# stjude-rust-labs/ngs

Measured on AMD Instinct MI355X. Metric: BAM records/sec (whole node), all qc facets, 150 bp reads, higher is better.
Workload: dtype u8/u32 integer (u64 accumulators)

## Files before the change

ngs_amd/csrc/cov_stream.hip:

```cpp
#include <hip/hip_runtime.h>

#include <type_traits>

#include "kernels.h"

namespace ngsq {

typedef unsigned long long u64;

constexpr uint32_t ST_THREADS = 256;
constexpr uint32_t ST_WAVES = ST_THREADS / 64;
constexpr uint32_t ST_W = 1024;
constexpr uint32_t ST_LIST = 232;
constexpr uint32_t ST_HOT_BINS = 64, ST_HOT_REP = 4, ST_HOT = ST_HOT_BINS * ST_HOT_REP;

__device__ __forceinline__ u64 st_key(int32_t rf, int32_t ps) {
    return rf < 0 ? 0xFFFFFFFF00000000ull : ((u64)(uint32_t)rf << 32) | (uint32_t)(ps + 1);
}
__device__ __forceinline__ bool st_valid(const DeviceState &st, int32_t rf, int32_t ps) {
    return rf >= 0 && (uint32_t)rf < st.n_refs && ps >= 0 && st.ref_depth_off[rf] != NO_DEPTH;
}

__global__ __launch_bounds__(256) void k_cov_plan_tiles(DeviceState st, DeviceBatch b, CovStreamArgs a) {
    NGSQ_FOREGROUND_WAVE();
    const uint64_t n_wt = (b.n + CS_TILE - 1) / CS_TILE;
    const uint64_t t = (uint64_t)blockIdx.x * blockDim.x + threadIdx.x;
    if (t == 0) {
        const u64 k0 = st_key(b.ref_id[0], b.pos[0]);
        if (k0 < *a.last_key) atomicAdd(&st.counters[C_COV_UNSORTED], 1ull);
        *a.last_key = st_key(b.ref_id[b.n - 1], b.pos[b.n - 1]);
    }
    const uint32_t lane = threadIdx.x & 63u;
    auto first_of = [&](int64_t u, int32_t &r, int32_t &p) {
        const bool ok = u >= 0 && (uint64_t)u < n_wt;
        r = ok ? b.ref_id[(uint64_t)u * CS_TILE] : -1;
        p = ok ? b.pos[(uint64_t)u * CS_TILE] : -1;
    };
    int32_t rf[4], ps[4];
    first_of((int64_t)t, rf[1], ps[1]);
    rf[0] = __shfl_up(rf[1], 1, 64), ps[0] = __shfl_up(ps[1], 1, 64);
    rf[2] = __shfl_down(rf[1], 1, 64), ps[2] = __shfl_down(ps[1], 1, 64);
    rf[3] = __shfl_down(rf[1], 2, 64), ps[3] = __shfl_down(ps[1], 2, 64);
    if (lane == 0) first_of((int64_t)t - 1, rf[0], ps[0]);
    if (lane == 63) first_of((int64_t)t + 1, rf[2], ps[2]);
    if (lane >= 62) first_of((int64_t)t + 2, rf[3], ps[3]);
    if (t >= n_wt) return;
    auto streamable = [&](int k) {
        return st_valid(st, rf[k], ps[k]) && rf[k + 1] == rf[k] && ps[k + 1] >= 0;
    };
    if (!streamable(1)) return;
    const bool prev_same = streamable(0) && rf[0] == rf[1];
    const bool next_same = streamable(2) && rf[2] == rf[1];
    if (!prev_same) atomicMin(&a.plan_a[rf[1]], (uint32_t)ps[1] + 1);
    if (!next_same) atomicMax(&a.plan_z[rf[1]], (uint32_t)ps[2] + 1);
}

__global__ __launch_bounds__(256) void k_cov_plan_refs(DeviceState st, CovStreamArgs a) {
    NGSQ_FOREGROUND_WAVE();
    const uint32_t r = blockIdx.x * blockDim.x + threadIdx.x;
    if (r == 0 && a.span_next) *a.span_next = 0;
    if (r >= st.n_refs) return;
    const uint32_t pa = a.plan_a[r], pz = a.plan_z[r], prev = a.prev_end[r];
    const uint32_t acc = st.end_acc[r];
    uint32_t guard = a.guard_until[r];
    if (a.head_guard && guard == 0 && (pa != CS_NONE || acc != 0)) {
        const uint64_t g = (uint64_t)(pa != CS_NONE ? pa : acc) + a.head_guard;
        guard = g > 0xFFFFFFFEull ? 0xFFFFFFFEu : (uint32_t)g;
        a.guard_until[r] = guard;
    }
    uint32_t H = CS_NONE, T = CS_NONE;
    if (pa != CS_NONE && pz > pa) {
        uint64_t base = pa > prev + 1 ? pa : (uint64_t)prev + 1;
        if (guard > base) base = guard;
        const uint64_t h = (base + COV_CHUNK - 1) / COV_CHUNK * COV_CHUNK;
        const uint64_t lim = pz < (uint64_t)st.ref_len[r] + 1 ? pz : (uint64_t)st.ref_len[r] + 1;
        const uint64_t tt = lim / COV_CHUNK * COV_CHUNK;
        if (h < tt) {
            H = (uint32_t)h;
            T = (uint32_t)tt;
        }
    }
    a.plan_h[r] = H;
    a.plan_t[r] = T;
    a.prev_end[r] = acc > prev ? acc : prev;
    a.plan_a[r] = CS_NONE;
    a.plan_z[r] = 0;
}

__device__ __forceinline__ uint32_t st_wave_scan(uint32_t v) {
    v += (uint32_t)__builtin_amdgcn_update_dpp(0, (int)v, 0x111, 0xF, 0xF, false);
    v += (uint32_t)__builtin_amdgcn_update_dpp(0, (int)v, 0x112, 0xF, 0xF, false);
    v += (uint32_t)__builtin_amdgcn_update_dpp(0, (int)v, 0x114, 0xF, 0xF, false);
    v += (uint32_t)__builtin_amdgcn_update_dpp(0, (int)v, 0x118, 0xF, 0xF, false);
    v += (uint32_t)__builtin_amdgcn_update_dpp(0, (int)v, 0x142, 0xA, 0xF, false);
    v += (uint32_t)__builtin_amdgcn_update_dpp(0, (int)v, 0x143, 0xC, 0xF, false);
    return v;
}
__device__ __forceinline__ uint32_t st_wave_max(uint32_t v) {
#pragma unroll
    for (int o = 32; o > 0; o >>= 1) v = max(v, (uint32_t)__shfl_xor(v, o, 64));
    return v;
}

__host__ __device__ inline uint32_t st_hist_words(uint32_t cov_cap) { return ((cov_cap + 2 + 1) / 2 + 3) & ~3u; }

constexpr uint32_t ST_PER_LANE = 8;
constexpr uint32_t ST_PASS = 64 * ST_PER_LANE;
static_assert(ST_W % ST_PASS == 0, "whole passes");

struct StTileIn {
    int4 p;
    uint4 c;
    int32_t rf_t, ps_t, rf_n, ps_n;
};

constexpr uint32_t ST_MIN_BLOCKS = 4;
__global__ __launch_bounds__(ST_THREADS, ST_MIN_BLOCKS) void k_cov_stream(DeviceState st, DeviceBatch b, CovStreamArgs a) {
    NGSQ_FOREGROUND_WAVE();
    extern __shared__ __attribute__((aligned(16))) uint32_t s_dyn[];
    const uint32_t nb = a.cov_cap + 2;
    const uint32_t tid = threadIdx.x, lane = tid & 63;
    const uint32_t wave = (uint32_t)__builtin_amdgcn_readfirstlane((int)(tid >> 6));
    const uint32_t hw = st_hist_words(a.cov_cap);
    uint32_t *const win = s_dyn + wave * (ST_W + hw + ST_HOT + ST_LIST);
    uint32_t *const hist = win + ST_W;
    uint32_t *const hot = hist + hw;
    uint32_t *const lst = hot + ST_HOT;
    for (uint32_t i = lane; i < ST_W + hw + ST_HOT + ST_LIST; i += 64) win[i] = 0;
    __builtin_amdgcn_fence(__ATOMIC_ACQ_REL, "wavefront");
    __builtin_amdgcn_wave_barrier();

    const uint64_t n_wt = (b.n + CS_TILE - 1) / CS_TILE;
    const uint64_t n_full = b.n / CS_TILE;
    const uint64_t n_units = (uint64_t)gridDim.x * ST_WAVES, unit = (uint64_t)blockIdx.x * ST_WAVES + wave;
    const uint64_t per = (n_wt + n_units - 1) / n_units;
    const uint64_t t_begin = per * unit < n_wt ? per * unit : n_wt;
    const uint64_t t_end = t_begin + per < n_wt ? t_begin + per : n_wt;
    const uint32_t maxspan = *st.batch_span;

    uint32_t hot_base = 0;
    int32_t hist_ref = -1;
    uint32_t since_flush = 0;
    u64 zero_run = 0;
    uint32_t lane_zero = 0;
    u64 *bins = a.bin_totals;
    u64 lane_bin = 0;
    uint32_t bin_q = 0, bin_p0 = 1, bin_p1 = 0;
    u64 t_lo = ~0ull, t_hi = 0;
    bool lst_valid = false;
    uint64_t lst_tile = 0;
    int32_t lst_ref = -1;
    uint32_t lst_lo = 0, lst_n = 0;
    int32_t plan_ref = -1;
    uint32_t pH = CS_NONE, pT = CS_NONE, pL = 0;
    uint64_t pOff = 0;

    auto flush_bin = [&]() {
        u64 v = lane_bin;
#pragma unroll
        for (int o = 32; o > 0; o >>= 1) v += __shfl_xor(v, o, 64);
        if (lane == 0 && v) atomicAdd(&bins[bin_q], v);
        lane_bin = 0;
    };
    auto flush_hot = [&]() {
        static_assert((ST_HOT_REP == 4 || ST_HOT_REP == 8) && ST_HOT_BINS <= 64, "one or two uint4 per lane");
        uint4 *const cell = reinterpret_cast<uint4 *>(hot) + (lane < ST_HOT_BINS ? lane : 0u) * (ST_HOT_REP / 4);
        uint32_t t = 0;
        if (lane < ST_HOT_BINS) {
#pragma unroll
            for (uint32_t q = 0; q < ST_HOT_REP / 4; q++) {
                const uint4 v = cell[q];
                cell[q] = make_uint4(0, 0, 0, 0);
                t += v.x + v.y + v.z + v.w;
            }
        }
        const uint32_t depth = hot_base + lane;
        const uint32_t bin = depth <= a.cov_cap ? depth : a.cov_cap + 1;
        if (t) atomicAdd(&hist[bin < hw ? bin : bin - hw], bin < hw ? t : t << 16);
        __builtin_amdgcn_fence(__ATOMIC_ACQ_REL, "wavefront");
        __builtin_amdgcn_wave_barrier();
    };
    auto flush_hist = [&]() {
        if (hist_ref < 0) return;
        flush_hot();
        u64 *dst = a.hist + (u64)hist_ref * nb;
        for (uint32_t i = lane; i < hw; i += 64) {
            const uint32_t v = hist[i];
            if (v) {
                if ((v & 0xFFFFu) && i < nb) atomicAdd(&dst[i], (u64)(v & 0xFFFFu));
                if ((v >> 16) && i + hw < nb) atomicAdd(&dst[i + hw], (u64)(v >> 16));
                hist[i] = 0;
            }
        }
        {
            u64 z = lane_zero;
#pragma unroll
            for (int o = 32; o > 0; o >>= 1) z += __shfl_xor(z, o, 64);
            if (lane == 0 && zero_run + z) atomicAdd(&dst[0], zero_run + z);
        }
        zero_run = 0;
        lane_zero = 0;
        since_flush = 0;
        __builtin_amdgcn_fence(__ATOMIC_ACQ_REL, "wavefront");
        __builtin_amdgcn_wave_barrier();
    };
    auto chunk_add = [&](bool active, uint64_t chunk, uint32_t val) {
        const u64 m = __ballot(active);
        if (!m) return;
        const uint32_t c0 = __shfl((uint32_t)chunk, __ffsll((long long)m) - 1, 64);
        const bool same = active && (uint32_t)chunk == c0;
        uint32_t sum = same ? val : 0u;
#pragma unroll
        for (int o = 32; o > 0; o >>= 1) sum += __shfl_xor(sum, o, 64);
        if (lane == 0 && sum) atomicAdd(&st.chunk_sums[c0], sum);
        if (active && !same) atomicAdd(&st.chunk_sums[chunk], val);
    };
    auto classic = [&](bool on, uint64_t off, uint32_t q0, uint32_t q1, bool minus_in_sum_only) {
        const uint64_t g0 = off + q0, g1 = off + q1;
        if (on) {
            atomicAdd(&st.depth[g0], 1u);
            if (!minus_in_sum_only) atomicAdd(&st.depth[g1], 0xFFFFFFFFu);
            t_lo = g0 < t_lo ? g0 : t_lo;
            t_hi = g1 + 1 > t_hi ? g1 + 1 : t_hi;
        }
        chunk_add(on, g0 / COV_CHUNK, 1u);
        chunk_add(on, g1 / COV_CHUNK, 0xFFFFFFFFu);
    };
    auto outside = [&](bool on, uint64_t off, uint32_t sj, uint32_t ej, uint32_t H, uint32_t T) {
        const bool head = on && sj < H;
        const uint32_t m = ej < H ? ej : H;
        if (__ballot(head)) classic(head, off, sj, m, m == H);
        const bool tl = on && T != CS_NONE && ej > T;
        if (__ballot(tl)) classic(tl, off, sj > T ? sj : T, ej, false);
    };

    auto load_full = [&](uint64_t t) -> StTileIn {
        const uint64_t base = t * CS_TILE, r0 = base + (uint64_t)lane * 4;
        StTileIn in;
        in.p = *reinterpret_cast<const int4 *>(b.pos + r0);
        in.c = *reinterpret_cast<const uint4 *>(st.cov_end + r0);
        const uint64_t nx = base + CS_TILE < b.n ? base + CS_TILE : base;
        in.rf_t = b.ref_id[base];
        in.ps_t = b.pos[base];
        in.rf_n = b.ref_id[nx];
        in.ps_n = b.pos[nx];
        return in;
    };

    auto process = [&](const StTileIn &in, uint64_t t) {
        const uint64_t base = t * CS_TILE;
        const uint64_t r0 = base + (uint64_t)lane * 4;
        const uint32_t s[4] = {(uint32_t)in.p.x + 1, (uint32_t)in.p.y + 1, (uint32_t)in.p.z + 1, (uint32_t)in.p.w + 1};
        const uint32_t e[4] = {in.c.x, in.c.y, in.c.z, in.c.w};
        const int32_t rf_t = __builtin_amdgcn_readfirstlane(in.rf_t), ps_t = __builtin_amdgcn_readfirstlane(in.ps_t);
        const int32_t rf_n = __builtin_amdgcn_readfirstlane(in.rf_n), ps_n = __builtin_amdgcn_readfirstlane(in.ps_n);
        const bool cand = base + CS_TILE < b.n && rf_t >= 0 && (uint32_t)rf_t < st.n_refs && ps_t >= 0 && rf_n == rf_t && ps_n >= 0;
        if (cand && rf_t != plan_ref) {
            plan_ref = rf_t;
            pH = (uint32_t)__builtin_amdgcn_readfirstlane((int)a.plan_h[rf_t]);
            pT = (uint32_t)__builtin_amdgcn_readfirstlane((int)a.plan_t[rf_t]);
            pL = (uint32_t)__builtin_amdgcn_readfirstlane((int)st.ref_len[rf_t]);
            const uint64_t o = st.ref_depth_off[rf_t];
            pOff = ((uint64_t)(uint32_t)__builtin_amdgcn_readfirstlane((int)(o >> 32)) << 32) |
                   (uint32_t)__builtin_amdgcn_readfirstlane((int)(uint32_t)o);
        }
        const bool streamable = cand && pOff != NO_DEPTH;
        const uint32_t H = streamable ? pH : CS_NONE, T = streamable ? pT : CS_NONE, Lr = pL;
        const uint64_t off = pOff;

        if (streamable) {
#pragma unroll
            for (uint32_t j = 0; j < 4; j++) {
                const uint32_t ej = e[j] < Lr + 1 ? e[j] : Lr + 1;
                const bool on = e[j] != 0 && s[j] < ej && (s[j] < H || ej > T);
                if (__ballot(on)) outside(on, off, s[j], ej, H, T);
            }
        } else {
            for (uint32_t j = 0; j < 4; j++) {
                const int32_t rj = e[j] != 0 ? b.ref_id[r0 + j] : -1;
                const bool okr = rj >= 0 && (uint32_t)rj < st.n_refs;
                const uint64_t oj = okr ? st.ref_depth_off[rj] : NO_DEPTH;
                const uint32_t Lj = okr ? st.ref_len[rj] : 0u;
                const uint32_t ej = e[j] < Lj + 1 ? e[j] : Lj + 1;
                const uint32_t hj = okr ? a.plan_h[rj] : CS_NONE, tj = okr ? a.plan_t[rj] : CS_NONE;
                const bool on = oj != NO_DEPTH && s[j] < ej;
                if (__ballot(on)) outside(on, oj == NO_DEPTH ? 0 : oj, s[j], ej, hj, tj);
            }
            return;
        }
        if (H == CS_NONE) return;
        const uint32_t lo = (uint32_t)ps_t + 1 > H ? (uint32_t)ps_t + 1 : H;
        const uint32_t hi = (uint32_t)ps_n + 1 < T ? (uint32_t)ps_n + 1 : T;
        if (lo >= hi) return;

        if (hist_ref != rf_t) {
            flush_hist();
            flush_bin();
            hist_ref = rf_t;
            bins = a.bin_totals + a.bin_off[rf_t];
            bin_p0 = 1;
            bin_p1 = 0;
        }
        for (uint64_t p = ((uint64_t)lo + COV_CHUNK - 1) / COV_CHUNK * COV_CHUNK + (uint64_t)lane * COV_CHUNK; p < hi;
             p += 64ull * COV_CHUNK)
            a.chunk_flags[(off + p) / COV_CHUNK] = 1;
        t_lo = off + lo < t_lo ? off + lo : t_lo;
        t_hi = off + hi > t_hi ? off + hi : t_hi;

        bool rec[4];
#pragma unroll
        for (uint32_t j = 0; j < 4; j++) rec[j] = e[j] > lo && s[j] < hi;
        const bool from_list = lst_valid && lst_tile == t && lst_ref == rf_t && lst_lo == lo;
        uint32_t new_n = 0;
        bool new_ok = true;
        uint32_t w = lo, carry = 0;
        uint32_t lb_reach = CS_NONE;
        uint32_t lb_lane = 0;
        bool first = true;
        while (w < hi) {
            const uint32_t wend = hi - w > ST_W ? w + ST_W : hi;
#pragma unroll
            for (uint32_t j = 0; j < 4; j++) {
                const uint32_t sp = s[j] > lo ? s[j] : lo;
                if (rec[j] && sp >= w && sp < wend) atomicAdd(&win[sp - w], 1u);
                if (rec[j] && e[j] >= w && e[j] < wend) atomicAdd(&win[e[j] - w], 0xFFFFFFFFu);
            }
            if (lb_reach >= w) {
                uint32_t reach = 0;
                if (from_list) {
                    if (first && lane == 0 && lst_n) atomicAdd(&win[0], lst_n);
                    for (uint32_t c = 0; c < lst_n; c += 64) {
                        const uint32_t ee = c + lane < lst_n ? lst[c + lane] : 0u;
                        if (ee >= w && ee < wend && ee > lo) atomicAdd(&win[ee - w], 0xFFFFFFFFu);
                        reach = ee > reach ? ee : reach;
                    }
                } else {
                    uint32_t cnt0 = 0;
                    bool more = true;
                    for (uint64_t back = 64; more; back += 64) {
                        const bool okl = base + lane >= back;
                        const uint64_t idx = okl ? base + lane - back : 0;
                        const int32_t rf0 = b.ref_id[base >= back ? base - back : 0];
                        const uint32_t ss = (uint32_t)b.pos[idx] + 1, ee = st.cov_end[idx];
                        bool same = okl;
                        if (base < back || rf0 != rf_t) same = same && b.ref_id[idx] == rf_t;
                        const bool hit = same && ee > lo;
                        if (first) {
                            cnt0 += (uint32_t)__popcll(__ballot(hit));
                            const u64 km = __ballot(hit && ee > hi);
                            const uint32_t kn = (uint32_t)__popcll(km);
                            if (new_n + kn <= ST_LIST) {
                                if (hit && ee > hi) lst[new_n + __builtin_amdgcn_mbcnt_hi((uint32_t)(km >> 32), __builtin_amdgcn_mbcnt_lo((uint32_t)km, 0))] = ee;
                                new_n += kn;
                            } else {
                                new_ok = false;
                            }
                        }
                        if (hit && ee >= w && ee < wend) atomicAdd(&win[ee - w], 0xFFFFFFFFu);
                        reach = hit && ee > reach ? ee : reach;
                        const uint32_t ss0 = (uint32_t)__builtin_amdgcn_readfirstlane((int)ss);
                        more = base > back && rf0 == rf_t && (uint64_t)ss0 + maxspan > lo;
                    }
                    if (first && lane == 0 && cnt0) atomicAdd(&win[0], cnt0);
                }
                lb_lane = reach;
            }
            __builtin_amdgcn_fence(__ATOMIC_ACQ_REL, "wavefront");
            __builtin_amdgcn_wave_barrier();

            const uint32_t len = wend - w;
            auto pass = [&](auto pl_tag, uint32_t pb) {
                constexpr uint32_t PL = decltype(pl_tag)::value;
                uint32_t x[PL];
                if constexpr (PL == 8) {
                    uint4 *cell = reinterpret_cast<uint4 *>(win + pb + lane * PL);
                    const uint4 d0 = cell[0], d1 = cell[1];
                    cell[0] = make_uint4(0, 0, 0, 0);
                    cell[1] = make_uint4(0, 0, 0, 0);
                    x[0] = d0.x, x[1] = d0.y, x[2] = d0.z, x[3] = d0.w, x[4] = d1.x, x[5] = d1.y, x[6] = d1.z, x[7] = d1.w;
                } else if constexpr (PL == 4) {
                    uint4 *cell = reinterpret_cast<uint4 *>(win + pb + lane * PL);
                    const uint4 d0 = cell[0];
                    cell[0] = make_uint4(0, 0, 0, 0);
                    x[0] = d0.x, x[1] = d0.y, x[2] = d0.z, x[3] = d0.w;
                } else {
                    uint2 *cell = reinterpret_cast<uint2 *>(win + pb + lane * PL);
                    const uint2 d0 = cell[0];
                    cell[0] = make_uint2(0, 0);
                    x[0] = d0.x, x[1] = d0.y;
                }
#pragma unroll
                for (uint32_t k = 1; k < PL; k++) x[k] += x[k - 1];
                if (carry - hot_base - ST_HOT_BINS / 8 >= 3 * ST_HOT_BINS / 4) {
                    const uint32_t nb0 = carry > ST_HOT_BINS / 2 ? carry - ST_HOT_BINS / 2 : 0u;
                    if (nb0 != hot_base) {
                        flush_hot();
                        hot_base = nb0;
                    }
                }
                const uint32_t hot_lane = (uint32_t)(hot - hist) + (lane & (ST_HOT_REP - 1)) - hot_base * ST_HOT_REP;
                const uint32_t inc = st_wave_scan(x[PL - 1]);
                const uint32_t before = carry + inc - x[PL - 1];
                carry += (uint32_t)__builtin_amdgcn_readlane((int)inc, 63);
                const uint32_t p_first = w + pb, p_last = (len - pb > 64 * PL ? p_first + 64 * PL - 1 : wend - 1);
                const bool one_bin = p_first >= bin_p0 && p_last < bin_p1;
                if (!one_bin) {
                    const uint32_t q0 = (p_first - 1) / a.bin_size, q1 = (p_last - 1) / a.bin_size;
                    if (q0 == q1) {
                        flush_bin();
                        bin_q = q0 + 1;
                        bin_p0 = q0 * a.bin_size + 1;
                        const uint64_t top = (uint64_t)(q0 + 1) * a.bin_size + 1;
                        bin_p1 = top > 0xFFFFFFFFull ? 0xFFFFFFFFu : (uint32_t)top;
                    }
                }
                const bool in_acc = p_first >= bin_p0 && p_last < bin_p1;
                uint32_t lsum = 0;
#pragma unroll
                for (uint32_t k = 0; k < PL; k++) {
                    const uint32_t i = pb + lane * PL + k;
                    const uint32_t depth = before + x[k];
                    const uint32_t bin = depth <= a.cov_cap ? depth : a.cov_cap + 1;
                    lane_zero += i < len && depth == 0;
                    const uint32_t one = i < len && depth != 0 ? 1u : 0u;
                    const bool in_hot = depth - hot_base < ST_HOT_BINS;
                    const uint32_t word = !one ? lane : in_hot ? hot_lane + depth * ST_HOT_REP : bin < hw ? bin : bin - hw;
                    atomicAdd(&hist[word], in_hot || bin < hw ? one : one << 16);
                    lsum += i < len ? depth : 0u;
                }
                if (in_acc) {
                    lane_bin += lsum;
                } else {
                    for (uint32_t k = 0; k < PL; k++) {
                        const uint32_t i = pb + lane * PL + k;
                        const uint32_t depth = before + x[k];
                        if (i < len && depth) atomicAdd(&bins[(u64)(w + i - 1) / a.bin_size + 1], (u64)depth);
                    }
                }
                since_flush += 64 * PL;
            };
            for (uint32_t pb = 0; pb < len;) {
                const uint32_t rem = len - pb;
                if (rem > 256) {
                    pass(std::integral_constant<uint32_t, 8>{}, pb);
                    pb += 512;
                } else if (rem > 128) {
                    pass(std::integral_constant<uint32_t, 4>{}, pb);
                    pb += 256;
                } else {
                    pass(std::integral_constant<uint32_t, 2>{}, pb);
                    pb += 128;
                }
            }
            if (since_flush > 0xFFFFu - 2 * ST_PASS) flush_hist();
            __builtin_amdgcn_fence(__ATOMIC_ACQ_REL, "wavefront");
            __builtin_amdgcn_wave_barrier();
            first = false;
            w = wend;
            if (w < hi) {
                lb_reach = st_wave_max(lb_lane);
                uint32_t reach = lb_reach, nxt = 0xFFFFFFFFu - hi;
#pragma unroll
                for (uint32_t j = 0; j < 4; j++) {
                    if (rec[j] && s[j] < w) reach = max(reach, e[j]);
                    if (rec[j] && s[j] >= w) nxt = max(nxt, 0xFFFFFFFFu - s[j]);
                }
                reach = st_wave_max(reach);
                nxt = 0xFFFFFFFFu - st_wave_max(nxt);
                if (reach <= w && nxt > w) {
                    zero_run += nxt - w;
                    carry = 0;
                    w = nxt;
                    __builtin_amdgcn_fence(__ATOMIC_ACQ_REL, "wavefront");
                    __builtin_amdgcn_wave_barrier();
                }
            }
        }

        if (from_list) {
            for (uint32_t c = 0; c < lst_n; c += 64) {
                const uint32_t ee = c + lane < lst_n ? lst[c + lane] : 0u;
                const u64 km = __ballot(ee > hi);
                if (ee > hi) lst[new_n + __builtin_amdgcn_mbcnt_hi((uint32_t)(km >> 32), __builtin_amdgcn_mbcnt_lo((uint32_t)km, 0))] = ee;
                new_n += (uint32_t)__popcll(km);
            }
        }
#pragma unroll
        for (uint32_t j = 0; j < 4; j++) {
            const u64 km = __ballot(e[j] > hi);
            const uint32_t kn = (uint32_t)__popcll(km);
            if (new_ok && new_n + kn <= ST_LIST) {
                if (e[j] > hi) lst[new_n + __builtin_amdgcn_mbcnt_hi((uint32_t)(km >> 32), __builtin_amdgcn_mbcnt_lo((uint32_t)km, 0))] = e[j];
                new_n += kn;
            } else {
                new_ok = false;
            }
        }
        lst_valid = new_ok;
        lst_n = new_n;
        lst_tile = t + 1;
        lst_ref = rf_t;
        lst_lo = hi;
        __builtin_amdgcn_fence(__ATOMIC_ACQ_REL, "wavefront");
        __builtin_amdgcn_wave_barrier();
    };

    uint64_t t = t_begin;
    const uint64_t t_full_end = t_end < n_full ? t_end : n_full;
    if (t < t_full_end) {
        StTileIn cur = load_full(t);
        while (t < t_full_end) {
            const uint64_t tn = t + 1;
            const StTileIn nxt = load_full(tn < n_full ? tn : t);
            process(cur, t);
            cur = nxt;
            t = tn;
        }
    }
    if (n_full < n_wt && t_begin <= n_full && n_full < t_end) {
        const uint64_t base = n_full * CS_TILE, r0 = base + (uint64_t)lane * 4;
        int32_t p[4];
        uint32_t c[4];
#pragma unroll
        for (uint32_t j = 0; j < 4; j++) {
            const bool ok = r0 + j < b.n;
            p[j] = ok ? b.pos[r0 + j] : -1;
            c[j] = ok ? st.cov_end[r0 + j] : 0u;
        }
        StTileIn in;
        in.p = make_int4(p[0], p[1], p[2], p[3]);
        in.c = make_uint4(c[0], c[1], c[2], c[3]);
        in.rf_t = in.rf_n = b.ref_id[base];
        in.ps_t = in.ps_n = b.pos[base];
        process(in, n_full);
    }
    flush_hist();
    flush_bin();
#pragma unroll
    for (int o = 32; o > 0; o >>= 1) {
        const u64 l2 = __shfl_xor(t_lo, o, 64), h2 = __shfl_xor(t_hi, o, 64);
        t_lo = l2 < t_lo ? l2 : t_lo;
        t_hi = h2 > t_hi ? h2 : t_hi;
    }
    if (lane == 0 && t_hi > 0) {
        atomicMin(&st.touched[0], t_lo);
        atomicMax(&st.touched[1], t_hi);
    }
}

hipError_t launch_cov_stream(const LaunchInfo &li, const DeviceState &st, const DeviceBatch &b, const CovStreamArgs &a,
                             hipStream_t s) {
    if (!b.n) return hipSuccess;
    const uint64_t n_wt = (b.n + CS_TILE - 1) / CS_TILE;
    hipLaunchKernelGGL(k_cov_plan_tiles, dim3((uint32_t)((n_wt + 255) / 256)), dim3(256), 0, s, st, b, a);
    hipLaunchKernelGGL(k_cov_plan_refs, dim3((st.n_refs + 255) / 256), dim3(256), 0, s, st, a);
    const size_t lds = (size_t)ST_WAVES * (ST_W + st_hist_words(a.cov_cap) + ST_HOT + ST_LIST) * sizeof(uint32_t);
    static bool attr = false;
    if (!attr) {
        hipError_t e = hipFuncSetAttribute(reinterpret_cast<const void *>(k_cov_stream),
                                           hipFuncAttributeMaxDynamicSharedMemorySize, 160 * 1024 - 64);
        if (e != hipSuccess) return e;
        attr = true;
    }
    uint64_t g = (n_wt + ST_WAVES - 1) / ST_WAVES;
    const uint64_t per_cu = (160 * 1024 - 1024) / lds;
    const uint64_t cap = (uint64_t)li.n_cu * (per_cu < 1 ? 1 : per_cu > 6 ? 6 : per_cu);
    if (g > cap) g = cap;
    hipLaunchKernelGGL(k_cov_stream, dim3((uint32_t)g), dim3(ST_THREADS), lds, s, st, b, a);
    return hipGetLastError();
}

}
```

Before: 18.45 billion.

## Replace LDS full depth histogram with per-lane relative-depth cells and global outliers

Drops the per-wave LDS histogram covering every depth up to cov_cap and the small hot window. Each wave now keeps a 128-bin window of depths around an exponentially smoothed running depth, stored as 32 per-lane replicated packed 16-bit counters to cut LDS atomic contention. Depths outside the window go straight to global memory through a ballot-grouped atomic path. This removes the LDS footprint that grew with cov_cap and the slow flush of the whole histogram, at the cost of extra global atomics when depth varies sharply, window re-centering flushes, and min-blocks lowered from 4 to 3.

```diff
diff --git a/ngs_amd/csrc/cov_stream.hip b/ngs_amd/csrc/cov_stream.hip
--- a/ngs_amd/csrc/cov_stream.hip
+++ b/ngs_amd/csrc/cov_stream.hip
@@ -12,7 +12,7 @@
 constexpr uint32_t ST_WAVES = ST_THREADS / 64;
 constexpr uint32_t ST_W = 1024;
 constexpr uint32_t ST_LIST = 232;
-constexpr uint32_t ST_HOT_BINS = 64, ST_HOT_REP = 4, ST_HOT = ST_HOT_BINS * ST_HOT_REP;
+constexpr uint32_t ST_HOT_BINS = 128, ST_CELLS = 64 * 32;
 
 __device__ __forceinline__ u64 st_key(int32_t rf, int32_t ps) {
     return rf < 0 ? 0xFFFFFFFF00000000ull : ((u64)(uint32_t)rf << 32) | (uint32_t)(ps + 1);
@@ -102,8 +102,6 @@
     return v;
 }
 
-__host__ __device__ inline uint32_t st_hist_words(uint32_t cov_cap) { return ((cov_cap + 2 + 1) / 2 + 3) & ~3u; }
-
 constexpr uint32_t ST_PER_LANE = 8;
 constexpr uint32_t ST_PASS = 64 * ST_PER_LANE;
 static_assert(ST_W % ST_PASS == 0, "whole passes");
@@ -114,19 +112,17 @@
     int32_t rf_t, ps_t, rf_n, ps_n;
 };
 
-constexpr uint32_t ST_MIN_BLOCKS = 4;
+constexpr uint32_t ST_MIN_BLOCKS = 3;
 __global__ __launch_bounds__(ST_THREADS, ST_MIN_BLOCKS) void k_cov_stream(DeviceState st, DeviceBatch b, CovStreamArgs a) {
     NGSQ_FOREGROUND_WAVE();
     extern __shared__ __attribute__((aligned(16))) uint32_t s_dyn[];
     const uint32_t nb = a.cov_cap + 2;
     const uint32_t tid = threadIdx.x, lane = tid & 63;
     const uint32_t wave = (uint32_t)__builtin_amdgcn_readfirstlane((int)(tid >> 6));
-    const uint32_t hw = st_hist_words(a.cov_cap);
-    uint32_t *const win = s_dyn + wave * (ST_W + hw + ST_HOT + ST_LIST);
-    uint32_t *const hist = win + ST_W;
-    uint32_t *const hot = hist + hw;
-    uint32_t *const lst = hot + ST_HOT;
-    for (uint32_t i = lane; i < ST_W + hw + ST_HOT + ST_LIST; i += 64) win[i] = 0;
+    uint32_t *const win = s_dyn + wave * (ST_W + ST_CELLS + ST_LIST);
+    uint32_t *const cells = win + ST_W;
+    uint32_t *const lst = cells + ST_CELLS;
+    for (uint32_t i = lane; i < ST_W + ST_CELLS + ST_LIST; i += 64) win[i] = 0;
     __builtin_amdgcn_fence(__ATOMIC_ACQ_REL, "wavefront");
     __builtin_amdgcn_wave_barrier();
 
@@ -139,6 +135,8 @@
     const uint32_t maxspan = *st.batch_span;
 
     uint32_t hot_base = 0;
+    uint32_t depth_avg = 0;
+    bool depth_fresh = true;
     int32_t hist_ref = -1;
     uint32_t since_flush = 0;
     u64 zero_run = 0;
@@ -162,47 +160,43 @@
         if (lane == 0 && v) atomicAdd(&bins[bin_q], v);
         lane_bin = 0;
     };
-    auto flush_hot = [&]() {
-        static_assert((ST_HOT_REP == 4 || ST_HOT_REP == 8) && ST_HOT_BINS <= 64, "one or two uint4 per lane");
-        uint4 *const cell = reinterpret_cast<uint4 *>(hot) + (lane < ST_HOT_BINS ? lane : 0u) * (ST_HOT_REP / 4);
-        uint32_t t = 0;
-        if (lane < ST_HOT_BINS) {
-#pragma unroll
-            for (uint32_t q = 0; q < ST_HOT_REP / 4; q++) {
-                const uint4 v = cell[q];
-                cell[q] = make_uint4(0, 0, 0, 0);
-                t += v.x + v.y + v.z + v.w;
-            }
-        }
-        const uint32_t depth = hot_base + lane;
-        const uint32_t bin = depth <= a.cov_cap ? depth : a.cov_cap + 1;
-        if (t) atomicAdd(&hist[bin < hw ? bin : bin - hw], bin < hw ? t : t << 16);
+    auto flush_cells = [&]() {
+        static_assert(ST_HOT_BINS == 128 && ST_CELLS == 2048, "two relative depths per lane");
+        if (hist_ref < 0) return;
         __builtin_amdgcn_fence(__ATOMIC_ACQ_REL, "wavefront");
         __builtin_amdgcn_wave_barrier();
-    };
-    auto flush_hist = [&]() {
-        if (hist_ref < 0) return;
-        flush_hot();
-        u64 *dst = a.hist + (u64)hist_ref * nb;
-        for (uint32_t i = lane; i < hw; i += 64) {
-            const uint32_t v = hist[i];
-            if (v) {
-                if ((v & 0xFFFFu) && i < nb) atomicAdd(&dst[i], (u64)(v & 0xFFFFu));
-                if ((v >> 16) && i + hw < nb) atomicAdd(&dst[i + hw], (u64)(v >> 16));
-                hist[i] = 0;
-            }
-        }
-        {
-            u64 z = lane_zero;
-#pragma unroll
-            for (int o = 32; o > 0; o >>= 1) z += __shfl_xor(z, o, 64);
-            if (lane == 0 && zero_run + z) atomicAdd(&dst[0], zero_run + z);
-        }
-        zero_run = 0;
-        lane_zero = 0;
+        const uint32_t *const row = cells + lane * 32;
+        uint32_t t = 0, t2 = 0;
+#pragma unroll 8
+        for (uint32_t k = 0; k < 32; k++) {
+            const uint32_t v = row[(k + lane) & 31];
+            t += v & 0xFFFFu;
+            t2 += v >> 16;
+        }
+        __builtin_amdgcn_fence(__ATOMIC_ACQ_REL, "wavefront");
+        __builtin_amdgcn_wave_barrier();
+#pragma unroll
+        for (uint32_t q = 0; q < ST_CELLS / 256; q++) reinterpret_cast<uint4 *>(cells)[q * 64 + lane] = make_uint4(0, 0, 0, 0);
+        u64 *const dst = a.hist + (u64)hist_ref * nb;
+        const uint32_t depth = hot_base + lane, depth2 = depth + 64;
+        if (t) atomicAdd(&dst[depth <= a.cov_cap ? depth : a.cov_cap + 1], (u64)t);
+        if (t2) atomicAdd(&dst[depth2 <= a.cov_cap ? depth2 : a.cov_cap + 1], (u64)t2);
         since_flush = 0;
         __builtin_amdgcn_fence(__ATOMIC_ACQ_REL, "wavefront");
         __builtin_amdgcn_wave_barrier();
+    };
+    auto flush_hist = [&]() {
+        if (hist_ref < 0) return;
+        flush_cells();
+        u64 *dst = a.hist + (u64)hist_ref * nb;
+        {
+            u64 z = lane_zero;
+#pragma unroll
+            for (int o = 32; o > 0; o >>= 1) z += __shfl_xor(z, o, 64);
+            if (lane == 0 && zero_run + z) atomicAdd(&dst[0], zero_run + z);
+        }
+        zero_run = 0;
+        lane_zero = 0;
     };
     auto chunk_add = [&](bool active, uint64_t chunk, uint32_t val) {
         const u64 m = __ballot(active);
@@ -297,6 +291,7 @@
             flush_hist();
             flush_bin();
             hist_ref = rf_t;
+            depth_fresh = true;
             bins = a.bin_totals + a.bin_off[rf_t];
             bin_p0 = 1;
             bin_p1 = 0;
@@ -391,16 +386,13 @@
                 }
 #pragma unroll
                 for (uint32_t k = 1; k < PL; k++) x[k] += x[k - 1];
-                if (carry - hot_base - ST_HOT_BINS / 8 >= 3 * ST_HOT_BINS / 4) {
-                    const uint32_t nb0 = carry > ST_HOT_BINS / 2 ? carry - ST_HOT_BINS / 2 : 0u;
-                    if (nb0 != hot_base) {
-                        flush_hot();
-                        hot_base = nb0;
-                    }
-                }
-                const uint32_t hot_lane = (uint32_t)(hot - hist) + (lane & (ST_HOT_REP - 1)) - hot_base * ST_HOT_REP;
                 const uint32_t inc = st_wave_scan(x[PL - 1]);
                 const uint32_t before = carry + inc - x[PL - 1];
+                if (depth_fresh) {
+                    depth_avg = carry + (uint32_t)__builtin_amdgcn_readfirstlane((int)x[0]);
+                    hot_base = depth_avg > ST_HOT_BINS / 2 ? depth_avg - ST_HOT_BINS / 2 : 0u;
+                    depth_fresh = false;
+                }
                 carry += (uint32_t)__builtin_amdgcn_readlane((int)inc, 63);
                 const uint32_t p_first = w + pb, p_last = (len - pb > 64 * PL ? p_first + 64 * PL - 1 : wend - 1);
                 const bool one_bin = p_first >= bin_p0 && p_last < bin_p1;
@@ -416,17 +408,34 @@
                 }
                 const bool in_acc = p_first >= bin_p0 && p_last < bin_p1;
                 uint32_t lsum = 0;
+                bool outlier = false;
+                uint32_t *const lane_cells = cells + (lane & 31);
 #pragma unroll
                 for (uint32_t k = 0; k < PL; k++) {
                     const uint32_t i = pb + lane * PL + k;
                     const uint32_t depth = before + x[k];
-                    const uint32_t bin = depth <= a.cov_cap ? depth : a.cov_cap + 1;
                     lane_zero += i < len && depth == 0;
-                    const uint32_t one = i < len && depth != 0 ? 1u : 0u;
-                    const bool in_hot = depth - hot_base < ST_HOT_BINS;
-                    const uint32_t word = !one ? lane : in_hot ? hot_lane + depth * ST_HOT_REP : bin < hw ? bin : bin - hw;
-                    atomicAdd(&hist[word], in_hot || bin < hw ? one : one << 16);
+                    const bool one = i < len && depth != 0;
+                    const uint32_t o = depth - hot_base;
+                    outlier |= one && o >= ST_HOT_BINS;
+                    atomicAdd(&lane_cells[(o & 63) * 32], one && o < ST_HOT_BINS ? 1u << ((o >> 2) & 16) : 0u);
                     lsum += i < len ? depth : 0u;
+                }
+                if (__ballot(outlier)) {
+                    u64 *const dst = a.hist + (u64)hist_ref * nb;
+                    for (uint32_t k = 0; k < PL; k++) {
+                        const uint32_t i = pb + lane * PL + k;
+                        const uint32_t depth = before + x[k];
+                        const uint32_t bin = depth <= a.cov_cap ? depth : a.cov_cap + 1;
+                        bool out = i < len && depth != 0 && depth - hot_base >= ST_HOT_BINS;
+                        for (u64 m = __ballot(out); m; m = __ballot(out)) {
+                            const uint32_t b0 = (uint32_t)__builtin_amdgcn_readlane((int)bin, __ffsll((long long)m) - 1);
+                            const bool same = out && bin == b0;
+                            const u64 ms = __ballot(same);
+                            if (lane == 0) atomicAdd(&dst[b0], (u64)__popcll(ms));
+                            out = out && !same;
+                        }
+                    }
                 }
                 if (in_acc) {
                     lane_bin += lsum;
@@ -437,7 +446,7 @@
                         if (i < len && depth) atomicAdd(&bins[(u64)(w + i - 1) / a.bin_size + 1], (u64)depth);
                     }
                 }
-                since_flush += 64 * PL;
+                since_flush += PL;
             };
             for (uint32_t pb = 0; pb < len;) {
                 const uint32_t rem = len - pb;
@@ -451,8 +460,14 @@
                     pass(std::integral_constant<uint32_t, 2>{}, pb);
                     pb += 128;
                 }
-            }
-            if (since_flush > 0xFFFFu - 2 * ST_PASS) flush_hist();
+                depth_avg += (uint32_t)(((int32_t)carry - (int32_t)depth_avg) >> 3);
+                const uint32_t nb0 = depth_avg > ST_HOT_BINS / 2 ? depth_avg - ST_HOT_BINS / 2 : 0u;
+                if (nb0 + ST_HOT_BINS / 8 - hot_base >= ST_HOT_BINS / 4) {
+                    flush_cells();
+                    hot_base = nb0;
+                }
+            }
+            if (since_flush > 0xFFFFu / 2 - 2 * ST_PER_LANE) flush_cells();
             __builtin_amdgcn_fence(__ATOMIC_ACQ_REL, "wavefront");
             __builtin_amdgcn_wave_barrier();
             first = false;
@@ -554,7 +569,7 @@
     const uint64_t n_wt = (b.n + CS_TILE - 1) / CS_TILE;
     hipLaunchKernelGGL(k_cov_plan_tiles, dim3((uint32_t)((n_wt + 255) / 256)), dim3(256), 0, s, st, b, a);
     hipLaunchKernelGGL(k_cov_plan_refs, dim3((st.n_refs + 255) / 256), dim3(256), 0, s, st, a);
-    const size_t lds = (size_t)ST_WAVES * (ST_W + st_hist_words(a.cov_cap) + ST_HOT + ST_LIST) * sizeof(uint32_t);
+    const size_t lds = (size_t)ST_WAVES * (ST_W + ST_CELLS + ST_LIST) * sizeof(uint32_t);
     static bool attr = false;
     if (!attr) {
         hipError_t e = hipFuncSetAttribute(reinterpret_cast<const void *>(k_cov_stream),
```

Result: no change. 18.42 billion (median of 4 runs) (-0.2%).
